# jayleicn/ClipBERT

Hardware: NVIDIA H100
Metric: clips/sec fwd+bwd MSRVTT ret (ResNet50+BERT-base) (higher is better)
Workload: dtype bf16

## Files before the change

clipbert_b200/_lib.py:

```python
import ctypes
import os

import torch

_HERE = os.path.dirname(os.path.abspath(__file__))
LIB_PATH = os.path.join(_HERE, "lib", "libclipbert_sm90.so")

CB_GEMM_TN, CB_GEMM_WGRAD = 0, 1
ACT_NONE, ACT_RELU, ACT_GELU, ACT_TANH, ACT_GELU_STASH_GRAD = 0, 1, 2, 3, 4
AUX_NONE, AUX_RELU_MASK, AUX_GELU_GRAD, AUX_TANH_GRAD, AUX_MUL = 0, 1, 2, 3, 4
ROWMAP_NONE, ROWMAP_PAD, ROWMAP_UNPAD = 0, 1, 2


class GemmDesc(ctypes.Structure):
    _fields_ = [
        ("mode", ctypes.c_int32),
        ("m", ctypes.c_int32), ("n", ctypes.c_int32), ("k", ctypes.c_int32),
        ("a", ctypes.c_void_p), ("a_rows", ctypes.c_int64), ("a_ld", ctypes.c_int64),
        ("b", ctypes.c_void_p), ("b_rows", ctypes.c_int64), ("b_ld", ctypes.c_int64),
        ("ntaps", ctypes.c_int32), ("tap_w", ctypes.c_int32), ("tap_sign", ctypes.c_int32),
        ("split_k", ctypes.c_int32),
        ("scale", ctypes.c_void_p), ("shift", ctypes.c_void_p),
        ("residual", ctypes.c_void_p), ("res_ld", ctypes.c_int64),
        ("aux", ctypes.c_void_p), ("aux_ld", ctypes.c_int64), ("aux_mode", ctypes.c_int32),
# ... 3 lines not shown
        ("rowmap", ctypes.c_int32), ("map_h", ctypes.c_int32), ("map_w", ctypes.c_int32),
        ("dropout_p", ctypes.c_float), ("dropout_seed", ctypes.c_uint64),
        ("block_n", ctypes.c_int32), ("reserved", ctypes.c_int32),
        ("workspace", ctypes.c_void_p), ("workspace_bytes", ctypes.c_int64),
    ]


class NativeLibraryMissing(RuntimeError):
    pass


_lib = None


def lib():
    global _lib
    if _lib is not None:
        return _lib
    if not os.path.exists(LIB_PATH):
        raise NativeLibraryMissing(
            "%s not found: run `python -c 'import __graft_entry__ as g; g.build()'` "
            "(there is no CPU / eager fallback for the ClipBERT hot path)" % LIB_PATH)
    L = ctypes.CDLL(LIB_PATH)
    L.cb_last_error.restype = ctypes.c_char_p
    L.cb_version.restype = ctypes.c_int
    L.cb_sm_arch.restype = ctypes.c_int
    L.cb_launch_count.restype = ctypes.c_int64
    L.cb_gemm.argtypes = [ctypes.POINTER(GemmDesc), ctypes.c_void_p]
    L.cb_gemm.restype = ctypes.c_int
    L.cb_gemm_wgrad_group.argtypes = [ctypes.POINTER(GemmDesc), ctypes.c_int, ctypes.c_void_p]
    L.cb_gemm_wgrad_group.restype = ctypes.c_int
    L.cb_gemm_tile_width.argtypes = [ctypes.POINTER(GemmDesc)]
    L.cb_gemm_tile_width.restype = ctypes.c_int
    L.cb_gemm_workspace_bytes.argtypes = [ctypes.POINTER(GemmDesc)]
    L.cb_gemm_workspace_bytes.restype = ctypes.c_int64
    L.cb_gemm_wgrad_group_workspace_bytes.argtypes = [ctypes.POINTER(GemmDesc), ctypes.c_int]
    L.cb_gemm_wgrad_group_workspace_bytes.restype = ctypes.c_int64
    L.cb_set_deterministic.argtypes = [ctypes.c_int]
    L.cb_set_deterministic.restype = ctypes.c_int
    _lib = L
    return L


def check(rc, what="cb call"):
    if rc != 0:
        raise RuntimeError("%s failed (%d): %s" % (what, rc, lib().cb_last_error().decode()))


def stream_ptr():
    return ctypes.c_void_p(torch.cuda.current_stream().cuda_stream)


def ptr(t):
    return None if t is None else t.data_ptr()
```

clipbert_b200/csrc/gemm.cu:

```cuda
#include <algorithm>

#include "common.cuh"
#include "host_util.h"

namespace cb {

constexpr int BM = 128;
constexpr int BK = 64;
constexpr int CONSUMER_WARPS = 8;
constexpr int GEMM_THREADS = (CONSUMER_WARPS + 1) * 32;
constexpr int PP_THREADS = 3 * 128;
constexpr int PP_PRODUCER_REGS = 40;
constexpr int PP_CONSUMER_REGS = 232;
constexpr int PP_BAR_TURN = 1;
constexpr int MAX_STAGES = 8;
constexpr int SMEM_LIMIT = 232448;
constexpr int STG_PITCH = 36;
constexpr int STG_WARP_FLOATS = 16 * STG_PITCH;
constexpr int EPI_BYTES = CONSUMER_WARPS * STG_WARP_FLOATS * 4;
constexpr int IN_BOX_BYTES = BM * 64 * 2;

struct GemmEpi {
  const float* scale;
  const float* shift;
  const __nv_bfloat16* residual;
  const __nv_bfloat16* aux;
  int aux_mode;
  int act;
  void* out;
  int64_t out_ld;
  int out_fp32;
  __nv_bfloat16* out2;
  int64_t out2_ld;
  int rowmap, H, W;
  uint32_t drop_thresh;
  float drop_inv_keep;
  uint64_t seed;
  const uint64_t* seed_off;
  int mn3d;
  long long* dbg;
};

__device__ __forceinline__ void dbg_stamp(const GemmEpi& epi, int slot) {
  if (epi.dbg) {
    epi.dbg[blockIdx.x * 32 + slot] = clock64();
    if (slot == 0 || slot == 11) {
      unsigned long long ns;
      asm volatile("mov.u64 %0, %%globaltimer;" : "=l"(ns));
      epi.dbg[blockIdx.x * 32 + (slot == 0 ? 12 : 13)] = static_cast<long long>(ns);
    }
  }
}

template <int BN>
struct GemmCfg {
  static constexpr int A_BYTES = BM * BK * 2;
  static constexpr int B_BYTES = BN * BK * 2;
  static constexpr int STAGE_BYTES = A_BYTES + B_BYTES;
  static constexpr int BAR_BYTES = 256;
};

enum { EK_GENERIC = 0, EK_SHIFT_ACT = 1, EK_RELU_MASK = 2, EK_DROP_RES = 3, EK_GELU_STASH = 4, EK_AUX_MUL = 5 };

__device__ __forceinline__ float relu_nan(float v) { return !(v <= 0.0f) ? v : 0.0f; }
__device__ __forceinline__ bool bf16_relu_pos(uint32_t x, bool lo) {
  const uint32_t b = lo ? (x & 0xffffu) : (x >> 16);
  return b - 0x0080u <= 0x7f80u - 0x0080u;
}

template <int NC>
__device__ __forceinline__ void add_shift(float (&f)[NC], const float (&shv)[NC]) {
#pragma unroll
  for (int j = 0; j < NC; ++j) f[j] += shv[j];
}
template <int NC>
__device__ __forceinline__ void add_residual(float (&f)[NC], const uint32_t (&res16)[NC / 2]) {
#pragma unroll
  for (int j = 0; j < NC / 2; ++j) {
    const float2 r2 = unpack_bf16x2(res16[j]);
    f[2 * j] += r2.x;
    f[2 * j + 1] += r2.y;
  }
}
template <int NC>
__device__ __forceinline__ void epilogue_shift_act(float (&f)[NC], const float (&shv)[NC], bool has_shift, const uint32_t (&res16)[NC / 2], bool has_res,
                                                   bool relu) {
  if (has_shift) add_shift<NC>(f, shv);
  if (has_res) add_residual<NC>(f, res16);
  if (relu) {
// ... 111 lines not shown
      case CB_AUX_GELU_GRAD:
#pragma unroll
        for (int j = 0; j < NC / 2; ++j) {
          const float2 a2 = unpack_bf16x2(aux16[j]);
          f[2 * j] *= gelu_erf_grad(a2.x);
          f[2 * j + 1] *= gelu_erf_grad(a2.y);
        }
        break;
      case CB_AUX_TANH_GRAD:
#pragma unroll
        for (int j = 0; j < NC / 2; ++j) {
          const float2 a2 = unpack_bf16x2(aux16[j]);
          f[2 * j] *= (1.0f - a2.x * a2.x);
          f[2 * j + 1] *= (1.0f - a2.y * a2.y);
        }
        break;
      case CB_AUX_MUL:
#pragma unroll
        for (int j = 0; j < NC / 2; ++j) {
          const float2 a2 = unpack_bf16x2(aux16[j]);
          f[2 * j] *= a2.x;
          f[2 * j + 1] *= a2.y;
        }
        break;
      default: break;
    }
  }
}

struct TileInfo {
  int m0, n0;
};

template <int BN>
__device__ __forceinline__ TileInfo decode_tile(int tile, int tiles_m, int tiles_n) {
  TileInfo t;
  t.m0 = (tile / tiles_n) % tiles_m * BM;
  t.n0 = tile % tiles_n * BN;
  return t;
}

template <int BN, int TA, int TB>
__device__ __forceinline__ void mma_tile(float (&acc)[BN / 2], uint32_t smem0, int stage_bytes, int KCH, int STAGES, int n_iters, int wg,
                                         int lane, int& s, uint32_t& ph, uint64_t* full_bar, uint64_t* empty_bar) {
  using Cfg = GemmCfg<BN>;
  int prev = -1;
  for (int i = 0; i < n_iters; i += KCH) {
    const int nch = min(KCH, n_iters - i);
    mbar_wait(&full_bar[s], ph);
    __syncwarp();
    wgmma_fence();
    wgmma_fence_acc(acc);
    for (int ch = 0; ch < nch; ++ch) {
      const uint32_t a_addr = smem0 + s * stage_bytes + ch * Cfg::STAGE_BYTES + wg * (64 * 128);
      const uint32_t b_addr = smem0 + s * stage_bytes + ch * Cfg::STAGE_BYTES + Cfg::A_BYTES;
#pragma unroll
      for (int k = 0; k < BK / 16; ++k) {
        const uint64_t ad = TA ? gmma_desc(a_addr + k * 2048, BK * 128, 1024) : gmma_desc(a_addr + k * 32, 16, 1024);
        const uint64_t bd = TB ? gmma_desc(b_addr + k * 2048, BK * 128, 1024) : gmma_desc(b_addr + k * 32, 16, 1024);
        wgmma_bf16<BN, TA, TB>(acc, ad, bd, (i > 0 || ch > 0 || k > 0) ? 1u : 0u);
      }
    }
    wgmma_commit();
    wgmma_wait<1>();
    wgmma_fence_acc(acc);
    if (prev >= 0) {
      __syncwarp();
      if (lane == 0) mbar_arrive(&empty_bar[prev]);
    }
    prev = s;
    if (++s == STAGES) { s = 0; ph ^= 1; }
  }
  wgmma_wait<0>();
  wgmma_fence_acc(acc);
  if (prev >= 0) {
    __syncwarp();
    if (lane == 0) mbar_arrive(&empty_bar[prev]);
  }
}

template <int BN, int TB>
__device__ __forceinline__ void mma_tile_pp(float (&acc)[2][BN / 2], uint32_t smem0, int stage_bytes, int KCH, int STAGES, int n_iters,
                                            int lane, int& s, uint32_t& ph, uint64_t* full_bar, uint64_t* empty_bar, int pass_bar,
                                            bool in_stage) {
  using Cfg = GemmCfg<BN>;
  int prev = -1;
  for (int i = 0; i < n_iters; i += KCH) {
    const int nch = min(KCH, n_iters - i);
    mbar_wait_unguarded(&full_bar[s], ph);
    __syncwarp();
    wgmma_fence();
    wgmma_fence_acc(acc[0]);
    wgmma_fence_acc(acc[1]);
    for (int ch = 0; ch < nch; ++ch) {
      const uint32_t a_addr = smem0 + s * stage_bytes + ch * Cfg::STAGE_BYTES;
      const uint32_t b_addr = a_addr + Cfg::A_BYTES;
#pragma unroll
      for (int k = 0; k < BK / 16; ++k) {
        const uint64_t bd = TB ? gmma_desc(b_addr + k * 2048, BK * 128, 1024) : gmma_desc(b_addr + k * 32, 16, 1024);
        const uint32_t accum = (i > 0 || ch > 0 || k > 0) ? 1u : 0u;
#pragma unroll
        for (int h = 0; h < 2; ++h) wgmma_bf16<BN, 0, TB>(acc[h], gmma_desc(a_addr + h * (64 * 128) + k * 32, 16, 1024), bd, accum);
      }
    }
    wgmma_commit();
    wgmma_wait<1>();
    wgmma_fence_acc(acc[0]);
    wgmma_fence_acc(acc[1]);
    if (prev >= 0) {
      __syncwarp();
      mbar_arrive_if(&empty_bar[prev], lane == 0);
    }
    prev = s;
    if (++s == STAGES) { s = 0; ph ^= 1; }
    if (pass_bar && i + KCH >= n_iters) {
      if (in_stage) mbar_wait_unguarded(&full_bar[s], ph);
      named_bar_arrive(pass_bar, 2 * 128);
    }
  }
  wgmma_wait<0>();
  wgmma_fence_acc(acc[0]);
  wgmma_fence_acc(acc[1]);
  if (prev >= 0) {
    __syncwarp();
    mbar_arrive_if(&empty_bar[prev], lane == 0);
  }
}

template <int BN, bool STORE = false>
__device__ __forceinline__ void wgrad_epilogue(const float (&acc)[BN / 2], float* obase, int64_t out_ld, const float* scale, int M, int N, int r0,
                                               int n0, int lane) {
  const int r1 = r0 + 8;
  const float rs0 = (r0 < M && scale) ? scale[r0] : 1.0f;
  const float rs1 = (r1 < M && scale) ? scale[r1] : 1.0f;
#pragma unroll
  for (int j = 0; j < BN / 8; ++j) {
    const int n = n0 + j * 8 + 2 * (lane & 3);
    if (n < N) {
      if constexpr (STORE) {
        if (r0 < M) *reinterpret_cast<float2*>(obase + static_cast<int64_t>(r0) * out_ld + n) = make_float2(acc[4 * j] * rs0, acc[4 * j + 1] * rs0);
        if (r1 < M) *reinterpret_cast<float2*>(obase + static_cast<int64_t>(r1) * out_ld + n) = make_float2(acc[4 * j + 2] * rs1, acc[4 * j + 3] * rs1);
      } else {
        if (r0 < M) red_add_f32x2(obase + static_cast<int64_t>(r0) * out_ld + n, acc[4 * j] * rs0, acc[4 * j + 1] * rs0);
        if (r1 < M) red_add_f32x2(obase + static_cast<int64_t>(r1) * out_ld + n, acc[4 * j + 2] * rs1, acc[4 * j + 3] * rs1);
      }
    }
  }
}

__device__ __forceinline__ uint32_t swz128(uint32_t box, int r, int q) { return box + r * 128 + ((q ^ (r & 7)) << 4); }

template <int BN, int MODE>
__device__ __forceinline__ void load_operand_stage(uint8_t* stage, const CUtensorMap* tmA, const CUtensorMap* tmB, uint64_t* bar, TileInfo t, int i,
                                                   int nch, int kc_per_tap, int K, int N, int ntaps, int tap_w, int tap_sign, int mn3d) {
  using Cfg = GemmCfg<BN>;
  constexpr int B_BOXES = (MODE == 0) ? 1 : BN / 64;
  int tp = 0, kc = i;
  if (ntaps > 1) { tp = i / kc_per_tap; kc = i - tp * kc_per_tap; }
  for (int ch = 0; ch < nch; ++ch) {
    uint8_t* sa = stage + ch * Cfg::STAGE_BYTES;
    uint8_t* sb = sa + Cfg::A_BYTES;
    int shift = 0;
    if (ntaps == 9) shift = tap_sign * ((tp / 3 - 1) * tap_w + (tp % 3 - 1));
    else if (ntaps > 1) shift = tap_sign * tp * tap_w;
    tma_load_2d(sa, tmA, bar, kc * BK, t.m0 + shift);
    if (MODE == 0) {
      tma_load_2d(sb, tmB, bar, tp * K + kc * BK, t.n0);
    } else if (mn3d) {
      tma_load_3d(sb, tmB, bar, 0, kc * BK, (tp * N + t.n0) >> 6);
    } else {
#pragma unroll
      for (int j = 0; j < B_BOXES; ++j) tma_load_2d(sb + j * (BK * 128), tmB, bar, tp * N + t.n0 + j * 64, kc * BK);
    }
    if (++kc == kc_per_tap) { kc = 0; ++tp; }
  }
}

__device__ __forceinline__ int output_row(const GemmEpi& epi, int m, int M) {
  bool row_ok = m < M;
  int64_t orow = m;
  if (epi.rowmap == CB_ROWMAP_PAD) {
    const int hw = epi.H * epi.W;
    const int img = m / hw;
    const int r = m - img * hw;
    const int y = r / epi.W, x = r - y * epi.W;
    orow = (static_cast<int64_t>(img) * (epi.H + 2) + y + 1) * (epi.W + 2) + x + 1;
  } else if (epi.rowmap == CB_ROWMAP_UNPAD) {
    const int wp = epi.W + 2, hp = epi.H + 2;
// ... 355 lines not shown
    mma_tile<BN, 0, MODE != 0>(acc, smem0, stage_bytes, KCH, STAGES, n_iters, wg, lane, s, ph, full_bar, empty_bar);
    const int orow = output_row(epi, t.m0 + brow, M);
#pragma unroll
    for (int j = 0; j < BN / 64; ++j) {
      if (n_in) mbar_wait_unguarded(&full_bar[s], ph);
      const uint32_t res_box = smem0 + s * stage_bytes;
      const uint32_t aux_box = res_box + (has_res ? IN_BOX_BYTES : 0);
#pragma unroll
      for (int h = 0; h < 2; ++h) {
        const int sc = 2 * j + h;
        __syncwarp();
#pragma unroll
        for (int jj = 0; jj < 4; ++jj) {
          const int f = sc * 4 + jj;
          float* p = stg + (lane >> 2) * STG_PITCH + jj * 8 + 2 * (lane & 3);
          *reinterpret_cast<float2*>(p) = make_float2(acc[4 * f], acc[4 * f + 1]);
          *reinterpret_cast<float2*>(p + 8 * STG_PITCH) = make_float2(acc[4 * f + 2], acc[4 * f + 3]);
        }
        __syncwarp();
        const int tc = sc * 32 + eh * 16;
        const int nb = t.n0 + tc;
        if (orow >= 0 && nb < N)
          epilogue_store16(epi, ek, dseed, smem_u32(stg + er * STG_PITCH + eh * 16), orow, nb, N, res_box, aux_box, brow, (tc & 63) >> 3);
      }
      if (n_in) {
        __syncwarp();
        mbar_arrive_if(&empty_bar[s], lane == 0);
        if (++s == STAGES) { s = 0; ph ^= 1; }
      }
    }
  }
}

static int g_sm_limit = 0;
static int sm_count_device() {
  static int n = 0;
  if (n == 0) {
    int dev = 0;
    cudaGetDevice(&dev);
    cudaDeviceGetAttribute(&n, cudaDevAttrMultiProcessorCount, dev);
    if (n <= 0) n = 132;
  }
  return n;
}
static int sm_count() {
  const int n = sm_count_device();
  return (g_sm_limit > 0 && g_sm_limit < n) ? g_sm_limit : n;
}
static int plan_sm_count() { return g_det.load(std::memory_order_relaxed) ? sm_count_device() : sm_count(); }

static long long* g_gemm_timeline = nullptr;
static int g_mn3d = 1;


struct SmemPlan {
  int epi_bytes, kch, stages, chunk_bytes, n_in;
};
static SmemPlan plan_ring(int bn, bool staging, int kiters, int force_kch, int in_bytes, int n_in) {
  SmemPlan p;
  const int limit = SMEM_LIMIT;
  p.chunk_bytes = BM * BK * 2 + bn * BK * 2;
  p.epi_bytes = staging ? EPI_BYTES : 0;
  p.n_in = n_in;
  const int chunks_fit = (limit - 1024 - GemmCfg<64>::BAR_BYTES - p.epi_bytes - n_in * in_bytes) / p.chunk_bytes;
  const int min_stages = kiters > chunks_fit ? 3 : 2;
  p.kch = 1;
  if (force_kch > 0) p.kch = force_kch;
  else if (kiters >= 4 && chunks_fit >= 4 * min_stages) p.kch = 4;
  else if (kiters >= 2 && chunks_fit >= 2 * min_stages) p.kch = 2;
  if (p.kch > kiters) p.kch = kiters;
  if (p.kch > 1 && chunks_fit / p.kch < 2) p.kch = 1;
  p.stages = chunks_fit / p.kch;
  if (p.stages > MAX_STAGES) p.stages = MAX_STAGES;
  const int stage_iters = ceil_div(kiters, p.kch);
  const int cap = staging ? 2 * stage_iters + 1 : (stage_iters + 1 > 2 ? stage_iters + 1 : 2);
  if (p.stages > cap) p.stages = cap;
  return p;
}
static SmemPlan plan_smem(int bn, bool staging, int kiters, int force_kch = 0, int in_bytes = 0) {
  if (staging && bn == 256) return plan_ring(bn, staging, kiters, force_kch, 0, 0);
  const SmemPlan none = plan_ring(bn, staging, kiters, force_kch, 0, 0);
  if (in_bytes == 0) return none;
  const SmemPlan two = plan_ring(bn, staging, kiters, force_kch, in_bytes, 2);
  if (two.stages >= 2 && two.stages * two.kch >= kiters) return two;
  if (kiters > 4 && none.stages >= 2 && none.kch * none.chunk_bytes >= in_bytes) return none;
  return plan_ring(bn, staging, kiters, force_kch, in_bytes, 1);
}
static int epi_in_bytes(const cb_gemm_desc& d, int bn) {
  return d.mode == CB_GEMM_WGRAD ? 0 : ((d.residual != nullptr) + (d.aux != nullptr)) * (bn / 64) * IN_BOX_BYTES;
}

static int real_splits(int kc, int want) {
  const int sp = want < 1 ? 1 : (want > kc ? kc : want);
  return ceil_div(kc, ceil_div(kc, sp));
}

struct SplitReduceJob {
  float* out;
  const float* ws;
  int64_t out_ld;
  int M, W, S;
};
struct SplitReduce {
  int njobs;
  SplitReduceJob j[8];
};
__global__ void __launch_bounds__(256) wgrad_split_reduce_kernel(const __grid_constant__ SplitReduce r) {
  pdl_wait();
  pdl_trigger();
  const SplitReduceJob& J = r.j[blockIdx.y];
  const int w4 = J.W / 4;
  const int64_t total = static_cast<int64_t>(J.M) * w4, plane = static_cast<int64_t>(J.M) * J.W;
  for (int64_t i = static_cast<int64_t>(blockIdx.x) * 256 + threadIdx.x; i < total; i += static_cast<int64_t>(gridDim.x) * 256) {
    const int64_t m = i / w4;
    const int c = static_cast<int>(i - m * w4) * 4;
    float4* o = reinterpret_cast<float4*>(J.out + m * J.out_ld + c);
    float4 v = *o;
    const float* p = J.ws + m * J.W + c;
    for (int s = 0; s < J.S; ++s) {
      const float4 a = *reinterpret_cast<const float4*>(p + s * plane);
      v.x += a.x; v.y += a.y; v.z += a.z; v.w += a.w;
    }
    *o = v;
  }
}
static int launch_split_reduce(const SplitReduce& r, cudaStream_t stream, const char* what) {
  int64_t most = 0;
  for (int i = 0; i < r.njobs; ++i) most = std::max(most, static_cast<int64_t>(r.j[i].M) * (r.j[i].W / 4));
  const int gx = static_cast<int>(std::min<int64_t>(1024, (most + 255) / 256));
  launch_k(wgrad_split_reduce_kernel, dim3(gx, r.njobs), 256, 0, stream, r);
  return check_launch(what);
}

template <int BN, int MODE>
static int launch_gemm(const cb_gemm_desc& d, const GemmEpi& epi_in, cudaStream_t stream) {
  GemmEpi epi = epi_in;
  using Cfg = GemmCfg<BN>;
  constexpr bool wide = BN == 256;
  static bool attr_set = false;
  const void* kern = wide ? reinterpret_cast<const void*>(gemm_coop_kernel<MODE>) : reinterpret_cast<const void*>(gemm_pingpong_kernel<wide ? 128 : BN, MODE>);
  if (!attr_set) {
    cudaError_t e = cudaFuncSetAttribute(kern, cudaFuncAttributeMaxDynamicSharedMemorySize, SMEM_LIMIT);
    if (e != cudaSuccess) {
      set_error("cudaFuncSetAttribute(smem=%d): %s", SMEM_LIMIT, cudaGetErrorString(e));
      return CB_ERR_CUDA;
    }
    attr_set = true;
  }
  alignas(64) CUtensorMap ta, tb, tr, tx;
  bool mn3d = false;
  const int tiles_m = ceil_div(d.m, BM), tiles_n = ceil_div(d.n, BN);
  const int total = tiles_m * tiles_n;
  const int kiters = ceil_div(d.k, BK) * d.ntaps;
  bool ok = get_tmap_2d(&ta, d.a, d.k, d.a_rows, d.a_ld, BK, BM);
  if (MODE == 0) {
    ok = ok && get_tmap_2d(&tb, d.b, static_cast<uint64_t>(d.k) * d.ntaps, d.b_rows, d.b_ld, BK, BN);
  } else {
    mn3d = g_mn3d && d.n % 64 == 0 &&
           get_tmap_3d_mn(&tb, d.b, static_cast<uint64_t>(d.n) * d.ntaps, d.b_rows, d.b_ld, BK, BN / 64);
    if (!mn3d) ok = ok && get_tmap_2d(&tb, d.b, static_cast<uint64_t>(d.n) * d.ntaps, d.b_rows, d.b_ld, 64, BK);
  }
  tr = ta;
  tx = ta;
  if (d.residual) ok = ok && get_tmap_2d(&tr, d.residual, d.n, d.m, d.res_ld, 64, BM);
  if (d.aux) ok = ok && get_tmap_2d(&tx, d.aux, d.n, d.m, d.aux_ld, 64, BM);
  if (!ok) return CB_ERR_CUDA;
  epi.mn3d = mn3d ? 1 : 0;
  const int units = sm_count();
  const int grid = total < units ? total : units;
  const int in_bytes = epi_in_bytes(d, BN);
  const SmemPlan sp = plan_smem(BN, true, kiters, (d.reserved >> 8) & 15, in_bytes);
  const int kch = sp.kch, stages = sp.stages;
  if (stages < 2) {
    set_error("cb_gemm: not enough shared memory for a 2-stage pipeline (BN=%d, epilogue %d B + inputs %d B)", BN, sp.epi_bytes,
              in_bytes);
    return CB_ERR_INVALID;
  }
  const int smem_bytes = stages * kch * Cfg::STAGE_BYTES + sp.n_in * in_bytes + sp.epi_bytes + Cfg::BAR_BYTES + 1024;
  if constexpr (wide)
    launch_gemm_k(gemm_coop_kernel<MODE>, grid, PP_THREADS, smem_bytes, stream, ta, tb, tr, tx, d.m, d.n, d.k, d.ntaps, d.tap_w, d.tap_sign,
                  tiles_m, tiles_n, total, stages, kch, epi);
  else
    launch_gemm_k(gemm_pingpong_kernel<BN, MODE>, grid, PP_THREADS, smem_bytes, stream, ta, tb, tr, tx, d.m, d.n, d.k, d.ntaps, d.tap_w,
                  d.tap_sign, tiles_m, tiles_n, total, stages, kch, sp.n_in, epi);
  return check_launch("cb_gemm");
}

struct LaunchCfg {
  int bn, splits;
};

static LaunchCfg choose_config(const cb_gemm_desc& d, int units) {
  const int kc = ceil_div(d.k, BK);
  const bool wgrad = d.mode == CB_GEMM_WGRAD;
  if (!wgrad && (d.reserved & CB_GEMM_FORCE_WIDE)) return {256, 1};
  const int block_n = (!wgrad && d.block_n == 256) ? 128 : d.block_n;
  const bool wide_ok = !wgrad && d.block_n == 0 && !(d.reserved & CB_GEMM_NO_WIDE);
  static const int cand[3] = {64, 128, 256};
  LaunchCfg best = {64, 1};
  double best_cost = 1e30;
  for (int c = 0; c < 3; ++c) {
    const int bn = cand[c];
    if (block_n && bn != block_n) continue;
    if (!wgrad && bn == 256 && !wide_ok) continue;
    if (bn > 64 && d.n <= bn / 2) continue;
    const int64_t base = static_cast<int64_t>(ceil_div(d.m, BM)) * ceil_div(d.n, bn) * (wgrad ? d.ntaps : 1);
    const int max_split = wgrad ? (d.split_k > 0 ? d.split_k : (kc < 32 ? kc : 32)) : 1;
    for (int sp = (wgrad && d.split_k > 0) ? d.split_k : 1; sp <= max_split; ++sp) {
      const int ips = ceil_div(wgrad ? kc : kc * d.ntaps, sp);
      const int real_sp = wgrad ? ceil_div(kc, ips) : 1;
      const int64_t tiles = base * real_sp;
      const double rounds = static_cast<double>((tiles + units - 1) / units);
      const SmemPlan pl = plan_smem(bn, !wgrad, ips, (d.reserved >> 8) & 15, epi_in_bytes(d, bn));
      if (pl.stages < 2) continue;
      const double shallow = (pl.stages * pl.kch < 3 && ips > 2) ? 3.0 : 1.0;
      const double stage_cost = 450.0 + pl.kch * pl.chunk_bytes / 60.0;
      const double main_loop = ceil_div(ips, pl.kch) * stage_cost * shallow;
      double cost;
      if (wgrad) {
        cost = rounds * (main_loop + bn * 24.0) + 2500.0;
      } else if (bn == 256) {
        cost = rounds * (main_loop + bn * 20.0 * (d.out2 ? 2.0 : 1.0)) + 2500.0;
      } else {
        const double epi = bn * 30.0;
        const double per_tile = main_loop > 0.5 * (main_loop + epi) ? main_loop : 0.5 * (main_loop + epi);
        cost = rounds * per_tile + 0.5 * epi + 2500.0;
      }
      if ((bn == 256 && !wgrad ? cost / 0.95 : cost) < best_cost) {
        best_cost = bn == 256 && !wgrad ? cost / 0.95 : cost;
        best = {bn, real_sp};
      }
    }
  }
  return best;
}

constexpr int WG_MAX_PROBLEMS = 8;
struct WgradProblem {
  CUtensorMap tmA, tmB;
  float* out;
  const float* scale;
  int64_t out_ld;
  int M, N, K;
  int ntaps, tap_w, tap_sign;
  int iters_per_split, tiles_m, tiles_n;
  int tile_begin;
  int mn3d;
};
struct WgradGroup {
  int nprob, total_tiles;
  WgradProblem p[WG_MAX_PROBLEMS];
};
struct WgradWorkspace {
  float* p[WG_MAX_PROBLEMS];
};
struct WgTile {
  int pi, m0, n0, tap, it_begin, n_iters;
};
__device__ __forceinline__ WgTile wg_decode(const WgradGroup& g, int tile) {
  WgTile t;
  int pi = 0;
  while (pi + 1 < g.nprob && tile >= g.p[pi + 1].tile_begin) ++pi;
  const WgradProblem& P = g.p[pi];
// ... 266 lines not shown
  epi.rowmap = d.rowmap;
  epi.H = d.map_h;
  epi.W = d.map_w;
  epi.seed = d.dropout_seed;
  epi.dbg = g_gemm_timeline;
  epi.mn3d = 0;
  {
    const DropCfg dc = make_drop(d.dropout_p, d.dropout_seed);
    epi.drop_thresh = dc.thresh;
    epi.drop_inv_keep = dc.inv_keep;
    epi.seed_off = dc.offset;
  }

  if (d.mode == CB_GEMM_TN || d.mode == CB_GEMM_NN) {
    const bool nn = d.mode == CB_GEMM_NN;
    CB_REQUIRE(d.n % 8 == 0, "cb_gemm(TN): n must be a multiple of 8 (got %d)", d.n);
    CB_REQUIRE(d.k % 8 == 0, "cb_gemm(TN): k must be a multiple of 8 (got %d)", d.k);
    CB_REQUIRE(d.out_ld % 8 == 0, "cb_gemm(TN): out_ld must be a multiple of 8");
    CB_REQUIRE(!d.residual || d.res_ld % 8 == 0, "cb_gemm(TN): res_ld must be a multiple of 8");
    CB_REQUIRE(!d.aux || d.aux_ld % 8 == 0, "cb_gemm(TN): aux_ld must be a multiple of 8");
    CB_REQUIRE((reinterpret_cast<uintptr_t>(d.residual) & 15) == 0, "cb_gemm(TN): residual must be 16-byte aligned");
    CB_REQUIRE((reinterpret_cast<uintptr_t>(d.aux) & 15) == 0, "cb_gemm(TN): aux must be 16-byte aligned");
    CB_REQUIRE((reinterpret_cast<uintptr_t>(d.a) & 15) == 0, "cb_gemm(TN): a must be 16-byte aligned");
    CB_REQUIRE((reinterpret_cast<uintptr_t>(d.b) & 15) == 0, "cb_gemm(TN): b must be 16-byte aligned");
    CB_REQUIRE((reinterpret_cast<uintptr_t>(d.out) & 15) == 0, "cb_gemm(TN): out must be 16-byte aligned");
    CB_REQUIRE((reinterpret_cast<uintptr_t>(d.out2) & 15) == 0, "cb_gemm(TN): out2 must be 16-byte aligned");
    CB_REQUIRE(!d.out2 || d.out2_ld % 8 == 0, "cb_gemm(TN): out2_ld must be a multiple of 8");
    CB_REQUIRE(!(d.out2 && d.out_fp32), "cb_gemm(TN): out2 requires a bf16 primary output");
    CB_REQUIRE(d.rowmap == CB_ROWMAP_NONE || (d.map_h > 0 && d.map_w > 0), "cb_gemm: rowmap needs map_h/map_w");
    CB_REQUIRE(d.ntaps == 1 || d.tap_w > 2, "cb_gemm: tap modes need tap_w (padded row pitch in pixels)");
    CB_REQUIRE(d.block_n == 0 || d.block_n == 64 || d.block_n == 128 || d.block_n == 256, "cb_gemm: block_n must be 0, 64, 128 or 256 (got %d)",
               d.block_n);
    const LaunchCfg lc = choose_config(d, sm_count());
    switch (lc.bn) {
      case 64: return nn ? launch_gemm<64, 2>(d, epi, stream) : launch_gemm<64, 0>(d, epi, stream);
      case 128: return nn ? launch_gemm<128, 2>(d, epi, stream) : launch_gemm<128, 0>(d, epi, stream);
      case 256: return nn ? launch_gemm<256, 2>(d, epi, stream) : launch_gemm<256, 0>(d, epi, stream);
      default: CB_REQUIRE(false, "cb_gemm: no tile width for block_n %d", d.block_n);
    }
  } else {
    const int rc = check_wgrad_desc(d, "cb_gemm(WGRAD)");
    if (rc != CB_OK) return rc;
    const LaunchCfg lc = choose_config(d, plan_sm_count());
    return launch_wgrad(&d, 1, lc.bn, lc.splits, stream, "cb_gemm");
  }
  return CB_ERR_INVALID;
}

extern "C" int cb_gemm_wgrad_group(const cb_gemm_desc* descs, int n, void* stream_v) {
  using namespace cb;
  CB_REQUIRE(descs != nullptr && n >= 1, "cb_gemm_wgrad_group: no problems");
  for (int i = 0; i < n; ++i) {
    char who[48];
    snprintf(who, sizeof(who), "cb_gemm_wgrad_group: problem %d", i);
    const int rc = check_wgrad_desc(descs[i], who);
    if (rc != CB_OK) return rc;
  }
  const GroupPlan gp = group_plan(descs, n, plan_sm_count());
  if (!gp.groupable) {
    for (int i = 0; i < n; ++i) {
      cb_gemm_desc d = descs[i];
      d.workspace = descs[0].workspace;
      d.workspace_bytes = descs[0].workspace_bytes;
      const int rc = cb_gemm(&d, stream_v);
      if (rc != CB_OK) return rc;
    }
    return CB_OK;
  }
  return launch_wgrad(descs, n, gp.bn, gp.split, static_cast<cudaStream_t>(stream_v), "cb_gemm_wgrad_group");
}

extern "C" int cb_gemm_tile_width(const cb_gemm_desc* d) {
  using namespace cb;
  if (d == nullptr || d->m <= 0 || d->n <= 0 || d->k <= 0) return 0;
  if (d->mode != CB_GEMM_WGRAD) return choose_config(*d, sm_count()).bn;
  return choose_config(*d, plan_sm_count()).bn;
}

extern "C" int64_t cb_gemm_workspace_bytes(const cb_gemm_desc* d) {
  using namespace cb;
  if (d == nullptr || d->mode != CB_GEMM_WGRAD || d->m <= 0 || d->n <= 0 || d->k <= 0) return 0;
  return wgrad_ws_bytes(*d, choose_config(*d, sm_count_device()).splits);
}

extern "C" int64_t cb_gemm_wgrad_group_workspace_bytes(const cb_gemm_desc* descs, int n) {
  using namespace cb;
  if (descs == nullptr || n < 1) return 0;
  for (int i = 0; i < n; ++i)
    if (descs[i].mode != CB_GEMM_WGRAD || descs[i].m <= 0 || descs[i].n <= 0 || descs[i].k <= 0) return 0;
  return group_ws_bytes(descs, n);
}
```

clipbert_b200/ops.py:

```python
import ctypes

import torch

from . import _lib as L
from ._lib import (ACT_GELU, ACT_GELU_STASH_GRAD, ACT_NONE, ACT_RELU, ACT_TANH, AUX_GELU_GRAD, AUX_MUL, AUX_NONE,
                   AUX_RELU_MASK, AUX_TANH_GRAD, CB_GEMM_TN, CB_GEMM_WGRAD, ROWMAP_NONE, ROWMAP_PAD, ROWMAP_UNPAD)

CB_GEMM_NN = 2
GEMM_FORCE_WIDE = 1 << 12
GEMM_NO_WIDE = 1 << 13
_c = ctypes
_vp, _i, _i64, _f, _u64 = _c.c_void_p, _c.c_int, _c.c_int64, _c.c_float, _c.c_uint64

_SIGS = {
    "cb_layernorm_fwd": [_vp, _vp, _vp, _vp, _vp, _i, _i, _f, _vp],
    "cb_layernorm_bwd": [_vp, _vp, _vp, _vp, _vp, _vp, _vp, _vp, _vp, _i, _i, _f, _u64, _vp],
    "cb_embed_text_fwd": [_vp, _vp, _vp, _vp, _vp, _vp, _vp, _vp, _i, _i, _i, _i, _i, _f, _f, _u64, _vp],
    "cb_embed_text_bwd": [_vp] * 12 + [_i, _i, _i, _i, _i, _f, _u64, _vp],
    "cb_embed_visual_fwd": [_vp, _vp, _i, _vp, _vp, _vp, _vp, _vp, _vp, _vp, _i, _i, _i, _i, _i, _i, _i, _f, _f, _u64, _vp],
    "cb_embed_visual_bwd": [_vp, _vp, _vp, _vp, _i] + [_vp] * 12 + [_i, _i, _i, _i, _i, _i, _i, _i, _f, _u64, _vp],
    "cb_colsum": [_vp, _i64, _vp, _i, _i, _vp],
    "cb_dropout": [_vp, _vp, _i64, _f, _u64, _vp],
    "cb_dropout_offset_advance": [_vp, _vp, _vp],
    "cb_gelu_bwd": [_vp, _vp, _vp, _i64, _vp],
    "cb_pad_cast": [_vp, _i64, _vp, _i, _i, _i, _vp],
    "cb_cast_scale": [_vp, _vp, _i64, _vp, _i64, _vp],
    "cb_cast_bf16_f32": [_vp, _vp, _i64, _vp],
    "cb_cast_scale_segments": [_vp, _vp, _vp, _i, _vp, _vp],
    "cb_nvls_allreduce_f32": [_vp, _i64, _i, _i, _f, _i, _vp],
    "cb_clip_lse_loss": [_vp, _vp, _vp, _vp, _i, _i, _i, _f, _vp],
    "cb_clip_pool_ce_loss": [_vp, _vp, _vp, _vp, _i, _i, _i, _i, _f, _vp],
    "cb_cross_entropy_fwd": [_vp, _i64, _vp, _vp, _vp, _i64, _i, _i64, _vp],
    "cb_cross_entropy_bwd": [_vp, _i64, _vp, _vp, _vp, _vp, _i64, _i64, _i, _i64, _vp],
    "cb_attention_fwd": [_vp, _i64, _vp, _vp, _i64, _vp, _i, _i, _i, _i, _i, _f, _u64, _vp],
    "cb_attention_bwd": [_vp, _i64, _vp, _vp, _vp, _i64, _vp, _vp, _i64, _i, _i, _i, _i, _i, _f, _u64, _vp],
    "cb_attention_probs": [_vp, _i64, _vp, _vp, _vp, _i, _i, _i, _i, _i, _f, _u64, _vp],
    "cb_attention_probs_bwd": [_vp, _i64, _vp, _vp, _vp, _vp, _vp, _i64, _i, _i, _i, _i, _i, _f, _u64, _vp],
    "cb_attention_dprobs": [_vp, _i64, _vp, _i64, _vp, _i, _i, _i, _i, _i, _vp],
    "cb_stem_im2col": [_vp, _i, _vp, _i, _i, _i, _i, _f, _f, _f, _vp],
    "cb_maxpool3x3s2": [_vp, _vp, _i, _i, _i, _i, _vp],
    "cb_maxpool3x3s2_strided": [_vp, _vp, _i, _i, _i, _i, _i64, _i64, _vp],
    "cb_maxpool3x3s2_bwd": [_vp, _vp, _vp, _i, _i, _i, _i, _vp],
    "cb_maxpool3x3s2_bwd_strided": [_vp, _vp, _vp, _i, _i, _i, _i, _i64, _i64, _vp],
# ... 206 lines not shown


def _tuned(kw):
    if _tuning is None:
        _load_tuning()
    if not _tuning or "block_n" in kw or "reserved" in kw:
        return kw
    t = _tuning.get(gemm_key(kw))
    if t is None:
        return kw
    bn, reserved = t[0], (t[2] << 8) | (32 if (len(t) > 3 and t[3]) else 0)
    if bn == 256 and kw.get("mode", CB_GEMM_TN) != CB_GEMM_WGRAD:
        bn, reserved = 0, reserved | GEMM_FORCE_WIDE
    return dict(kw, block_n=bn, split_k=t[1], reserved=reserved)


def _gemm_descs(kws):
    arr = (L.GemmDesc * len(kws))()
    for d, kw in zip(arr, kws):
        d.ntaps = 1
        d.tap_sign = 1
        d.split_k = 0
        for k, v in kw.items():
            if k in _GEMM_PTR_FIELDS:
                v = _p(v) if isinstance(v, torch.Tensor) else v
            setattr(d, k, v)
    return arr


def gemm_tile_width(kw):
    return int(L.lib().cb_gemm_tile_width(_gemm_descs([_tuned(kw)])))


def gemm_workspace_bytes(kw):
    return int(L.lib().cb_gemm_workspace_bytes(_gemm_descs([kw])))


def gemm_wgrad_group_workspace_bytes(kws):
    return int(L.lib().cb_gemm_wgrad_group_workspace_bytes(_gemm_descs(kws), len(kws)))


def _with_workspace(kw, nbytes):
    if nbytes <= 0:
        return kw
    ws, nb = _scratch_args(nbytes, kw["out"])
    return dict(kw, workspace=ws, workspace_bytes=nb)


def _launch_gemm(name, kws):
    arr = _gemm_descs(kws)
    timing = _gemm_timing is not None or _op_timing is not None
    if timing:
        e0, e1 = torch.cuda.Event(enable_timing=True), torch.cuda.Event(enable_timing=True)
        e0.record()
    if name == "cb_gemm":
        rc = L.lib().cb_gemm(arr, _s())
    else:
        rc = L.lib().cb_gemm_wgrad_group(arr, len(kws), _s())
    if rc != 0:
        raise RuntimeError("%s failed (%d): %s" % (name, rc, L.lib().cb_last_error().decode()))
    if timing:
        e1.record()
        if _gemm_timing is not None:
            _gemm_timing.append((e0, e1))
        if _op_timing is not None:
            d = arr[0]
# ... 288 lines not shown
```

include/clipbert_b200.h:

```cpp
#ifndef CLIPBERT_B200_H_
#define CLIPBERT_B200_H_

#include <stddef.h>
#include <stdint.h>

#ifdef __cplusplus
extern "C" {
#endif

typedef enum cb_status {
  CB_OK = 0,
  CB_ERR_INVALID = -1,
  CB_ERR_CUDA = -2,
  CB_ERR_UNSUPPORTED = -3
} cb_status;

const char* cb_last_error(void);
int cb_version(void);
int cb_sm_arch(void);
int64_t cb_launch_count(void);
int cb_set_pdl(int enable);

int cb_set_deterministic(int enable);

// ... 21 lines not shown
typedef struct cb_gemm_desc {
  int32_t mode;
  int32_t m, n, k;
  const void* a;
  int64_t a_rows, a_ld;
  const void* b;
  int64_t b_rows, b_ld;
  int32_t ntaps, tap_w, tap_sign;
  int32_t split_k;
  const float* scale;
  const float* shift;
  const void* residual;
  int64_t res_ld;
  const void* aux;
  int64_t aux_ld;
  int32_t aux_mode;
  int32_t act;
  void* out;
  int64_t out_ld;
  int32_t out_fp32;
  void* out2;
  int64_t out2_ld;
  int32_t rowmap, map_h, map_w;
  float dropout_p;
  uint64_t dropout_seed;
  int32_t block_n;
  int32_t reserved;
  void* workspace;
  int64_t workspace_bytes;
} cb_gemm_desc;

#define CB_GEMM_FORCE_WIDE (1 << 12)
#define CB_GEMM_NO_WIDE (1 << 13)

int cb_gemm(const cb_gemm_desc* desc, void* stream);
int cb_gemm_tile_width(const cb_gemm_desc* desc);
int64_t cb_gemm_workspace_bytes(const cb_gemm_desc* desc);
int cb_gemm_wgrad_group(const cb_gemm_desc* descs, int n, void* stream);
int64_t cb_gemm_wgrad_group_workspace_bytes(const cb_gemm_desc* descs, int n);

int cb_layernorm_fwd(const void* x, const float* gamma, const float* beta, void* y, float* stats, int m, int hidden,
                     float eps, void* stream);
int cb_layernorm_bwd(const void* dy, const void* x, const float* stats, const float* gamma, void* dx, void* dx_drop,
                     float* dgamma, float* dbeta, float* dbias_drop, int m, int hidden, float dropout_p,
                     uint64_t dropout_seed, void* stream);
int64_t cb_layernorm_bwd_scratch_bytes(int m);
int cb_layernorm_bwd_det(const void* dy, const void* x, const float* stats, const float* gamma, void* dx, void* dx_drop,
                         float* dgamma, float* dbeta, float* dbias_drop, int m, int hidden, float dropout_p,
                         uint64_t dropout_seed, float* scratch, int64_t scratch_bytes, void* stream);

int cb_embed_text_fwd(const int64_t* ids, const float* word, const float* pos, const float* type0, const float* gamma,
                      const float* beta, void* out, float* stats, int nseq, int lt, int l, int vocab, int hidden,
                      float eps, float dropout_p, uint64_t seed, void* stream);
int cb_embed_text_bwd(const void* dh, const int64_t* ids, const float* word, const float* pos, const float* type0,
                      const float* gamma, const float* stats, float* dword, float* dpos, float* dtype0, float* dgamma,
                      float* dbeta, int nseq, int lt, int l, int vocab, int hidden, float dropout_p, uint64_t seed,
                      void* stream);
int cb_embed_visual_fwd(const void* grid, const int32_t* seq2vid, int n_ex, const float* rowemb, const float* colemb,
                        const float* type0, const float* gamma, const float* beta, void* out, float* stats, int nseq,
                        int t, int gh, int gw, int lt, int l, int hidden, float eps, float dropout_p, uint64_t seed,
                        void* stream);
int cb_embed_visual_bwd(const void* dh, const void* grid, const int32_t* seq2vid, const int32_t* vid_start, int n_ex,
                        const float* rowemb, const float* colemb, const float* type0, const float* gamma,
                        const float* stats, float* dv_tmp, void* dgrid, float* drow, float* dcol, float* dtype0,
                        float* dgamma, float* dbeta, int nseq, int nvid, int t, int gh, int gw, int lt, int l, int hidden,
                        float dropout_p, uint64_t seed, void* stream);
int64_t cb_embed_text_bwd_scratch_bytes(int nseq, int lt);
int cb_embed_text_bwd_det(const void* dh, const int64_t* ids, const float* word, const float* pos, const float* type0,
                          const float* gamma, const float* stats, float* dword, float* dpos, float* dtype0, float* dgamma,
// ... 80 lines not shown
```

Baseline: 4115.

## Add cooperative 256-row GEMM tile kernel and include it in tile selection

Adds a gemm_tall_kernel in which two consumer warpgroups share a 256-row A tile and one B tile, so each loaded B tile serves twice as many output rows and per-output operand traffic drops. The cost model in choose_config now scores 256x64 and 256x128 tall tiles and also penalises non-coop NN GEMMs that carry an aux input, which can change which tile is chosen for existing shapes. The tall tile fills fewer SMs on small M and leaves fewer pipeline stages in shared memory, so the heuristic may pick it where it is not better.

```diff
diff --git a/clipbert_b200/_lib.py b/clipbert_b200/_lib.py
--- a/clipbert_b200/_lib.py
+++ b/clipbert_b200/_lib.py
@@ -59,6 +59,8 @@
     L.cb_gemm_wgrad_group.restype = ctypes.c_int
     L.cb_gemm_tile_width.argtypes = [ctypes.POINTER(GemmDesc)]
     L.cb_gemm_tile_width.restype = ctypes.c_int
+    L.cb_gemm_tile_shape.argtypes = [ctypes.POINTER(GemmDesc), ctypes.POINTER(ctypes.c_int)]
+    L.cb_gemm_tile_shape.restype = ctypes.c_int
     L.cb_gemm_workspace_bytes.argtypes = [ctypes.POINTER(GemmDesc)]
     L.cb_gemm_workspace_bytes.restype = ctypes.c_int64
     L.cb_gemm_wgrad_group_workspace_bytes.argtypes = [ctypes.POINTER(GemmDesc), ctypes.c_int]
diff --git a/clipbert_b200/csrc/gemm.cu b/clipbert_b200/csrc/gemm.cu
--- a/clipbert_b200/csrc/gemm.cu
+++ b/clipbert_b200/csrc/gemm.cu
@@ -52,9 +52,9 @@
   }
 }
 
-template <int BN>
+template <int BN, int ROWS = BM>
 struct GemmCfg {
-  static constexpr int A_BYTES = BM * BK * 2;
+  static constexpr int A_BYTES = ROWS * BK * 2;
   static constexpr int B_BYTES = BN * BK * 2;
   static constexpr int STAGE_BYTES = A_BYTES + B_BYTES;
   static constexpr int BAR_BYTES = 256;
@@ -232,10 +232,10 @@
   int m0, n0;
 };
 
-template <int BN>
+template <int BN, int ROWS = BM>
 __device__ __forceinline__ TileInfo decode_tile(int tile, int tiles_m, int tiles_n) {
   TileInfo t;
-  t.m0 = (tile / tiles_n) % tiles_m * BM;
+  t.m0 = (tile / tiles_n) % tiles_m * ROWS;
   t.n0 = tile % tiles_n * BN;
   return t;
 }
@@ -279,11 +279,11 @@
   }
 }
 
-template <int BN, int TB>
+template <int BN, int TB, int ROWS = BM>
 __device__ __forceinline__ void mma_tile_pp(float (&acc)[2][BN / 2], uint32_t smem0, int stage_bytes, int KCH, int STAGES, int n_iters,
                                             int lane, int& s, uint32_t& ph, uint64_t* full_bar, uint64_t* empty_bar, int pass_bar,
-                                            bool in_stage) {
-  using Cfg = GemmCfg<BN>;
+                                            bool in_stage, int a_row0 = 0) {
+  using Cfg = GemmCfg<BN, ROWS>;
   int prev = -1;
   for (int i = 0; i < n_iters; i += KCH) {
     const int nch = min(KCH, n_iters - i);
@@ -293,8 +293,9 @@
     wgmma_fence_acc(acc[0]);
     wgmma_fence_acc(acc[1]);
     for (int ch = 0; ch < nch; ++ch) {
-      const uint32_t a_addr = smem0 + s * stage_bytes + ch * Cfg::STAGE_BYTES;
-      const uint32_t b_addr = a_addr + Cfg::A_BYTES;
+      const uint32_t stage = smem0 + s * stage_bytes + ch * Cfg::STAGE_BYTES;
+      const uint32_t a_addr = stage + a_row0 * 128;
+      const uint32_t b_addr = stage + Cfg::A_BYTES;
 #pragma unroll
       for (int k = 0; k < BK / 16; ++k) {
         const uint64_t bd = TB ? gmma_desc(b_addr + k * 2048, BK * 128, 1024) : gmma_desc(b_addr + k * 32, 16, 1024);
@@ -350,10 +351,10 @@
 
 __device__ __forceinline__ uint32_t swz128(uint32_t box, int r, int q) { return box + r * 128 + ((q ^ (r & 7)) << 4); }
 
-template <int BN, int MODE>
+template <int BN, int MODE, int ROWS = BM>
 __device__ __forceinline__ void load_operand_stage(uint8_t* stage, const CUtensorMap* tmA, const CUtensorMap* tmB, uint64_t* bar, TileInfo t, int i,
                                                    int nch, int kc_per_tap, int K, int N, int ntaps, int tap_w, int tap_sign, int mn3d) {
-  using Cfg = GemmCfg<BN>;
+  using Cfg = GemmCfg<BN, ROWS>;
   constexpr int B_BOXES = (MODE == 0) ? 1 : BN / 64;
   int tp = 0, kc = i;
   if (ntaps > 1) { tp = i / kc_per_tap; kc = i - tp * kc_per_tap; }
@@ -775,6 +776,133 @@
   }
 }
 
+template <int BN, int MODE>
+__global__ void __launch_bounds__(PP_THREADS, 1)
+    gemm_tall_kernel(const __grid_constant__ CUtensorMap tmA, const __grid_constant__ CUtensorMap tmB, const __grid_constant__ CUtensorMap tmR,
+                     const __grid_constant__ CUtensorMap tmX, int M, int N, int K, int ntaps, int tap_w, int tap_sign, int tiles_m, int tiles_n,
+                     int total_tiles, int STAGES, int KCH, GemmEpi epi) {
+  static_assert(MODE != 1 && BN <= 128, "TN / NN tiles of 256 x 64 or 256 x 128");
+  constexpr int ROWS = 2 * BM;
+  constexpr int IN_BYTES = 2 * IN_BOX_BYTES;
+  using Cfg = GemmCfg<BN, ROWS>;
+  extern __shared__ uint8_t smem_raw[];
+  uint8_t* smem = reinterpret_cast<uint8_t*>((reinterpret_cast<uintptr_t>(smem_raw) + 1023) & ~static_cast<uintptr_t>(1023));
+  const int stage_bytes = KCH * Cfg::STAGE_BYTES;
+  const bool has_res = epi.residual != nullptr, has_aux = epi.aux != nullptr;
+  const int n_in = has_res + has_aux;
+  uint8_t* stg_base = smem + STAGES * stage_bytes;
+  uint64_t* full_bar = reinterpret_cast<uint64_t*>(stg_base + EPI_BYTES);
+  uint64_t* empty_bar = full_bar + MAX_STAGES;
+
+  const int warp = __shfl_sync(0xffffffffu, static_cast<int>(threadIdx.x >> 5), 0);
+  const int lane = threadIdx.x & 31;
+  const int unit = blockIdx.x, n_units = gridDim.x;
+  pdl_trigger();
+  if (threadIdx.x == 0) {
+    tma_prefetch_desc(&tmA);
+    tma_prefetch_desc(&tmB);
+    if (has_res) tma_prefetch_desc(&tmR);
+    if (has_aux) tma_prefetch_desc(&tmX);
+    for (int s = 0; s < STAGES; ++s) {
+      mbar_init(&full_bar[s], 1);
+      mbar_init(&empty_bar[s], CONSUMER_WARPS);
+    }
+    fence_mbar_init();
+  }
+  __syncthreads();
+  const int kc_per_tap = (K + BK - 1) / BK;
+  const int n_iters = ntaps * kc_per_tap;
+  pdl_wait();
+
+  if (warp < 4) {
+    setmaxnreg_dec<PP_PRODUCER_REGS>();
+    if (warp == 0 && lane == 0) {
+      int s = 0;
+      uint32_t ph = 0;
+      for (int tile = unit; tile < total_tiles; tile += n_units) {
+        const TileInfo t = decode_tile<BN, ROWS>(tile, tiles_m, tiles_n);
+        for (int i = 0; i < n_iters; i += KCH) {
+          const int nch = min(KCH, n_iters - i);
+          mbar_wait(&empty_bar[s], ph ^ 1);
+          mbar_expect_tx(&full_bar[s], nch * Cfg::STAGE_BYTES);
+          load_operand_stage<BN, MODE, ROWS>(smem + s * stage_bytes, &tmA, &tmB, &full_bar[s], t, i, nch, kc_per_tap, K, N, ntaps, tap_w,
+                                             tap_sign, epi.mn3d);
+          if (++s == STAGES) { s = 0; ph ^= 1; }
+        }
+        for (int j = 0; n_in && j < BN / 64; ++j) {
+          mbar_wait(&empty_bar[s], ph ^ 1);
+          mbar_expect_tx(&full_bar[s], n_in * IN_BYTES);
+          uint8_t* dst = smem + s * stage_bytes;
+#pragma unroll
+          for (int r = 0; r < 2; ++r) {
+            if (has_res) tma_load_2d(dst + r * IN_BOX_BYTES, &tmR, &full_bar[s], t.n0 + j * 64, t.m0 + r * BM);
+            if (has_aux) tma_load_2d(dst + (has_res ? IN_BYTES : 0) + r * IN_BOX_BYTES, &tmX, &full_bar[s], t.n0 + j * 64, t.m0 + r * BM);
+          }
+          if (++s == STAGES) { s = 0; ph ^= 1; }
+        }
+      }
+    }
+    return;
+  }
+
+  setmaxnreg_inc<PP_CONSUMER_REGS>();
+  const int wg = (warp >> 2) - 1;
+  const int wq = warp & 3;
+  const uint32_t smem0 = smem_u32(smem);
+  const uint64_t dseed = epi.drop_thresh ? drop_seed(epi.seed, epi.seed_off) : 0ull;
+  const EpiKind ek = epilogue_kind(epi, N);
+  const int er = lane & 15, eh = lane >> 4;
+  float* stg = reinterpret_cast<float*>(stg_base) + (warp - 4) * STG_WARP_FLOATS;
+  float acc[2][BN / 2];
+  int s = 0;
+  uint32_t ph = 0;
+  for (int tile = unit; tile < total_tiles; tile += n_units) {
+    const TileInfo t = decode_tile<BN, ROWS>(tile, tiles_m, tiles_n);
+    mma_tile_pp<BN, MODE != 0, ROWS>(acc, smem0, stage_bytes, KCH, STAGES, n_iters, lane, s, ph, full_bar, empty_bar, 0, false, wg * BM);
+    if (n_in) {
+      for (int j = 0; j < BN / 64; ++j) {
+        int sj = s + j;
+        const uint32_t pj = sj >= STAGES ? ph ^ 1u : ph;
+        mbar_wait_unguarded(&full_bar[sj >= STAGES ? sj - STAGES : sj], pj);
+      }
+    }
+#pragma unroll
+    for (int sc = 0; sc < BN / 32; ++sc) {
+#pragma unroll 1
+      for (int h = 0; h < 2; ++h) {
+        const int wrow = h * 64 + wq * 16;
+        __syncwarp();
+#pragma unroll
+        for (int jj = 0; jj < 4; ++jj) {
+          const int f = sc * 4 + jj;
+          float* p = stg + (lane >> 2) * STG_PITCH + jj * 8 + 2 * (lane & 3);
+          const bool h1 = h != 0;
+          *reinterpret_cast<float2*>(p) = make_float2(h1 ? acc[1][4 * f] : acc[0][4 * f], h1 ? acc[1][4 * f + 1] : acc[0][4 * f + 1]);
+          *reinterpret_cast<float2*>(p + 8 * STG_PITCH) =
+              make_float2(h1 ? acc[1][4 * f + 2] : acc[0][4 * f + 2], h1 ? acc[1][4 * f + 3] : acc[0][4 * f + 3]);
+        }
+        __syncwarp();
+        const int tc = sc * 32 + eh * 16;
+        const int nb = t.n0 + tc;
+        const int orow = output_row(epi, t.m0 + wg * BM + wrow + er, M);
+        if (orow < 0 || nb >= N) continue;
+        const int sj = s + (tc >> 6);
+        const uint32_t res_box = smem0 + (sj >= STAGES ? sj - STAGES : sj) * stage_bytes;
+        epilogue_store16(epi, ek, dseed, smem_u32(stg + er * STG_PITCH + eh * 16), orow, nb, N, res_box,
+                         res_box + (has_res ? IN_BYTES : 0), wg * BM + wrow + er, (tc & 63) >> 3);
+      }
+    }
+    if (n_in) {
+      __syncwarp();
+#pragma unroll
+      for (int j = 0; j < BN / 64; ++j) {
+        mbar_arrive_if(&empty_bar[s], lane == 0);
+        if (++s == STAGES) { s = 0; ph ^= 1; }
+      }
+    }
+  }
+}
+
 static int g_sm_limit = 0;
 static int sm_count_device() {
   static int n = 0;
@@ -799,10 +927,10 @@
 struct SmemPlan {
   int epi_bytes, kch, stages, chunk_bytes, n_in;
 };
-static SmemPlan plan_ring(int bn, bool staging, int kiters, int force_kch, int in_bytes, int n_in) {
+static SmemPlan plan_ring(int bn, bool staging, int kiters, int force_kch, int in_bytes, int n_in, int rows = BM) {
   SmemPlan p;
   const int limit = SMEM_LIMIT;
-  p.chunk_bytes = BM * BK * 2 + bn * BK * 2;
+  p.chunk_bytes = rows * BK * 2 + bn * BK * 2;
   p.epi_bytes = staging ? EPI_BYTES : 0;
   p.n_in = n_in;
   const int chunks_fit = (limit - 1024 - GemmCfg<64>::BAR_BYTES - p.epi_bytes - n_in * in_bytes) / p.chunk_bytes;
@@ -820,8 +948,8 @@
   if (p.stages > cap) p.stages = cap;
   return p;
 }
-static SmemPlan plan_smem(int bn, bool staging, int kiters, int force_kch = 0, int in_bytes = 0) {
-  if (staging && bn == 256) return plan_ring(bn, staging, kiters, force_kch, 0, 0);
+static SmemPlan plan_smem(int bn, bool staging, int kiters, int force_kch = 0, int in_bytes = 0, int rows = BM) {
+  if (staging && (bn == 256 || rows > BM)) return plan_ring(bn, staging, kiters, force_kch, 0, 0, rows);
   const SmemPlan none = plan_ring(bn, staging, kiters, force_kch, 0, 0);
   if (in_bytes == 0) return none;
   const SmemPlan two = plan_ring(bn, staging, kiters, force_kch, in_bytes, 2);
@@ -875,13 +1003,16 @@
   return check_launch(what);
 }
 
-template <int BN, int MODE>
+template <int BN, int MODE, int ROWS = BM>
 static int launch_gemm(const cb_gemm_desc& d, const GemmEpi& epi_in, cudaStream_t stream) {
   GemmEpi epi = epi_in;
-  using Cfg = GemmCfg<BN>;
-  constexpr bool wide = BN == 256;
+  using Cfg = GemmCfg<BN, ROWS>;
+  constexpr bool wide = BN == 256, tall = ROWS > BM;
+  static_assert(!(wide && tall), "no 256 x 256 tile");
   static bool attr_set = false;
-  const void* kern = wide ? reinterpret_cast<const void*>(gemm_coop_kernel<MODE>) : reinterpret_cast<const void*>(gemm_pingpong_kernel<wide ? 128 : BN, MODE>);
+  const void* kern = wide   ? reinterpret_cast<const void*>(gemm_coop_kernel<MODE>)
+                     : tall ? reinterpret_cast<const void*>(gemm_tall_kernel<wide ? 128 : BN, MODE>)
+                            : reinterpret_cast<const void*>(gemm_pingpong_kernel<wide ? 128 : BN, MODE>);
   if (!attr_set) {
     cudaError_t e = cudaFuncSetAttribute(kern, cudaFuncAttributeMaxDynamicSharedMemorySize, SMEM_LIMIT);
     if (e != cudaSuccess) {
@@ -892,10 +1023,10 @@
   }
   alignas(64) CUtensorMap ta, tb, tr, tx;
   bool mn3d = false;
-  const int tiles_m = ceil_div(d.m, BM), tiles_n = ceil_div(d.n, BN);
+  const int tiles_m = ceil_div(d.m, ROWS), tiles_n = ceil_div(d.n, BN);
   const int total = tiles_m * tiles_n;
   const int kiters = ceil_div(d.k, BK) * d.ntaps;
-  bool ok = get_tmap_2d(&ta, d.a, d.k, d.a_rows, d.a_ld, BK, BM);
+  bool ok = get_tmap_2d(&ta, d.a, d.k, d.a_rows, d.a_ld, BK, ROWS);
   if (MODE == 0) {
     ok = ok && get_tmap_2d(&tb, d.b, static_cast<uint64_t>(d.k) * d.ntaps, d.b_rows, d.b_ld, BK, BN);
   } else {
@@ -912,7 +1043,7 @@
   const int units = sm_count();
   const int grid = total < units ? total : units;
   const int in_bytes = epi_in_bytes(d, BN);
-  const SmemPlan sp = plan_smem(BN, true, kiters, (d.reserved >> 8) & 15, in_bytes);
+  const SmemPlan sp = plan_smem(BN, true, kiters, (d.reserved >> 8) & 15, in_bytes, ROWS);
   const int kch = sp.kch, stages = sp.stages;
   if (stages < 2) {
     set_error("cb_gemm: not enough shared memory for a 2-stage pipeline (BN=%d, epilogue %d B + inputs %d B)", BN, sp.epi_bytes,
@@ -923,6 +1054,9 @@
   if constexpr (wide)
     launch_gemm_k(gemm_coop_kernel<MODE>, grid, PP_THREADS, smem_bytes, stream, ta, tb, tr, tx, d.m, d.n, d.k, d.ntaps, d.tap_w, d.tap_sign,
                   tiles_m, tiles_n, total, stages, kch, epi);
+  else if constexpr (tall)
+    launch_gemm_k(gemm_tall_kernel<BN, MODE>, grid, PP_THREADS, smem_bytes, stream, ta, tb, tr, tx, d.m, d.n, d.k, d.ntaps, d.tap_w,
+                  d.tap_sign, tiles_m, tiles_n, total, stages, kch, epi);
   else
     launch_gemm_k(gemm_pingpong_kernel<BN, MODE>, grid, PP_THREADS, smem_bytes, stream, ta, tb, tr, tx, d.m, d.n, d.k, d.ntaps, d.tap_w,
                   d.tap_sign, tiles_m, tiles_n, total, stages, kch, sp.n_in, epi);
@@ -931,6 +1065,7 @@
 
 struct LaunchCfg {
   int bn, splits;
+  int rows = BM;
 };
 
 static LaunchCfg choose_config(const cb_gemm_desc& d, int units) {
@@ -939,39 +1074,46 @@
   if (!wgrad && (d.reserved & CB_GEMM_FORCE_WIDE)) return {256, 1};
   const int block_n = (!wgrad && d.block_n == 256) ? 128 : d.block_n;
   const bool wide_ok = !wgrad && d.block_n == 0 && !(d.reserved & CB_GEMM_NO_WIDE);
-  static const int cand[3] = {64, 128, 256};
+  const bool tall_fits = !wgrad && !(d.residual && d.aux);
+  if (tall_fits && (d.reserved & CB_GEMM_FORCE_TALL)) return {block_n ? block_n : (d.n > 64 ? 128 : 64), 1, 2 * BM};
+  const bool tall_ok = tall_fits && d.block_n == 0 && !(d.reserved & CB_GEMM_NO_TALL);
+  static const int cand[5][2] = {{64, BM}, {128, BM}, {256, BM}, {64, 2 * BM}, {128, 2 * BM}};
   LaunchCfg best = {64, 1};
   double best_cost = 1e30;
-  for (int c = 0; c < 3; ++c) {
-    const int bn = cand[c];
+  for (int c = 0; c < 5; ++c) {
+    const int bn = cand[c][0], rows = cand[c][1];
+    const bool coop = !wgrad && (bn == 256 || rows > BM);
     if (block_n && bn != block_n) continue;
     if (!wgrad && bn == 256 && !wide_ok) continue;
+    if (rows > BM && !tall_ok) continue;
     if (bn > 64 && d.n <= bn / 2) continue;
-    const int64_t base = static_cast<int64_t>(ceil_div(d.m, BM)) * ceil_div(d.n, bn) * (wgrad ? d.ntaps : 1);
+    const int64_t base = static_cast<int64_t>(ceil_div(d.m, rows)) * ceil_div(d.n, bn) * (wgrad ? d.ntaps : 1);
     const int max_split = wgrad ? (d.split_k > 0 ? d.split_k : (kc < 32 ? kc : 32)) : 1;
     for (int sp = (wgrad && d.split_k > 0) ? d.split_k : 1; sp <= max_split; ++sp) {
       const int ips = ceil_div(wgrad ? kc : kc * d.ntaps, sp);
       const int real_sp = wgrad ? ceil_div(kc, ips) : 1;
       const int64_t tiles = base * real_sp;
       const double rounds = static_cast<double>((tiles + units - 1) / units);
-      const SmemPlan pl = plan_smem(bn, !wgrad, ips, (d.reserved >> 8) & 15, epi_in_bytes(d, bn));
+      const SmemPlan pl = plan_smem(bn, !wgrad, ips, (d.reserved >> 8) & 15, epi_in_bytes(d, bn), rows);
       if (pl.stages < 2) continue;
       const double shallow = (pl.stages * pl.kch < 3 && ips > 2) ? 3.0 : 1.0;
       const double stage_cost = 450.0 + pl.kch * pl.chunk_bytes / 60.0;
-      const double main_loop = ceil_div(ips, pl.kch) * stage_cost * shallow;
+      double main_loop = ceil_div(ips, pl.kch) * stage_cost * shallow;
+      if (!wgrad && !coop && d.mode == CB_GEMM_NN && d.aux) main_loop *= 1.3;
+      if (rows > BM) main_loop *= 1.1;
       double cost;
       if (wgrad) {
         cost = rounds * (main_loop + bn * 24.0) + 2500.0;
-      } else if (bn == 256) {
-        cost = rounds * (main_loop + bn * 20.0 * (d.out2 ? 2.0 : 1.0)) + 2500.0;
+      } else if (coop) {
+        cost = rounds * (main_loop + (rows / BM) * bn * 20.0 * (d.out2 ? 2.0 : 1.0)) + 2500.0;
       } else {
         const double epi = bn * 30.0;
         const double per_tile = main_loop > 0.5 * (main_loop + epi) ? main_loop : 0.5 * (main_loop + epi);
         cost = rounds * per_tile + 0.5 * epi + 2500.0;
       }
-      if ((bn == 256 && !wgrad ? cost / 0.95 : cost) < best_cost) {
-        best_cost = bn == 256 && !wgrad ? cost / 0.95 : cost;
-        best = {bn, real_sp};
+      if ((coop ? cost / 0.95 : cost) < best_cost) {
+        best_cost = coop ? cost / 0.95 : cost;
+        best = {bn, real_sp, rows};
       }
     }
   }
@@ -1304,6 +1446,10 @@
     CB_REQUIRE(d.block_n == 0 || d.block_n == 64 || d.block_n == 128 || d.block_n == 256, "cb_gemm: block_n must be 0, 64, 128 or 256 (got %d)",
                d.block_n);
     const LaunchCfg lc = choose_config(d, sm_count());
+    if (lc.rows > BM) {
+      if (lc.bn == 64) return nn ? launch_gemm<64, 2, 2 * BM>(d, epi, stream) : launch_gemm<64, 0, 2 * BM>(d, epi, stream);
+      return nn ? launch_gemm<128, 2, 2 * BM>(d, epi, stream) : launch_gemm<128, 0, 2 * BM>(d, epi, stream);
+    }
     switch (lc.bn) {
       case 64: return nn ? launch_gemm<64, 2>(d, epi, stream) : launch_gemm<64, 0>(d, epi, stream);
       case 128: return nn ? launch_gemm<128, 2>(d, epi, stream) : launch_gemm<128, 0>(d, epi, stream);
@@ -1342,12 +1488,16 @@
   return launch_wgrad(descs, n, gp.bn, gp.split, static_cast<cudaStream_t>(stream_v), "cb_gemm_wgrad_group");
 }
 
-extern "C" int cb_gemm_tile_width(const cb_gemm_desc* d) {
+extern "C" int cb_gemm_tile_shape(const cb_gemm_desc* d, int* rows) {
   using namespace cb;
+  if (rows) *rows = 0;
   if (d == nullptr || d->m <= 0 || d->n <= 0 || d->k <= 0) return 0;
-  if (d->mode != CB_GEMM_WGRAD) return choose_config(*d, sm_count()).bn;
-  return choose_config(*d, plan_sm_count()).bn;
-}
+  const LaunchCfg lc = choose_config(*d, d->mode != CB_GEMM_WGRAD ? sm_count() : plan_sm_count());
+  if (rows) *rows = lc.rows;
+  return lc.bn;
+}
+
+extern "C" int cb_gemm_tile_width(const cb_gemm_desc* d) { return cb_gemm_tile_shape(d, nullptr); }
 
 extern "C" int64_t cb_gemm_workspace_bytes(const cb_gemm_desc* d) {
   using namespace cb;
diff --git a/clipbert_b200/ops.py b/clipbert_b200/ops.py
--- a/clipbert_b200/ops.py
+++ b/clipbert_b200/ops.py
@@ -9,6 +9,8 @@
 CB_GEMM_NN = 2
 GEMM_FORCE_WIDE = 1 << 12
 GEMM_NO_WIDE = 1 << 13
+GEMM_FORCE_TALL = 1 << 14
+GEMM_NO_TALL = 1 << 15
 _c = ctypes
 _vp, _i, _i64, _f, _u64 = _c.c_void_p, _c.c_int, _c.c_int64, _c.c_float, _c.c_uint64
 
@@ -281,6 +283,12 @@
     return int(L.lib().cb_gemm_tile_width(_gemm_descs([_tuned(kw)])))
 
 
+def gemm_tile_shape(kw):
+    rows = ctypes.c_int(0)
+    cols = L.lib().cb_gemm_tile_shape(_gemm_descs([_tuned(kw)]), ctypes.byref(rows))
+    return int(rows.value), int(cols)
+
+
 def gemm_workspace_bytes(kw):
     return int(L.lib().cb_gemm_workspace_bytes(_gemm_descs([kw])))
 
diff --git a/include/clipbert_b200.h b/include/clipbert_b200.h
--- a/include/clipbert_b200.h
+++ b/include/clipbert_b200.h
@@ -77,9 +77,12 @@
 
 #define CB_GEMM_FORCE_WIDE (1 << 12)
 #define CB_GEMM_NO_WIDE (1 << 13)
+#define CB_GEMM_FORCE_TALL (1 << 14)
+#define CB_GEMM_NO_TALL (1 << 15)
 
 int cb_gemm(const cb_gemm_desc* desc, void* stream);
 int cb_gemm_tile_width(const cb_gemm_desc* desc);
+int cb_gemm_tile_shape(const cb_gemm_desc* desc, int* rows);
 int64_t cb_gemm_workspace_bytes(const cb_gemm_desc* desc);
 int cb_gemm_wgrad_group(const cb_gemm_desc* descs, int n, void* stream);
 int64_t cb_gemm_wgrad_group_workspace_bytes(const cb_gemm_desc* descs, int n);
```

Result: no change. 4119 (median of 6 runs) (+0.1%).
